# maxsonate/video-diffusion-nnx

Measured on AMD Instinct MI355X. Metric: denoised frames/sec, 16fx64x64 1000-step DDPM, higher is better.
Workload: dtype bf16; 1 GPU; config_v2_2 (north-star shape): Unet3D dim=64 C=1, 16f x 64x64, DDPM T=1000 p_sample_loop (UNet forward + p_sample per step, hipGraph replay); value = n_gpus*B*F/(T*s_per_step); batch_per_gpu=64, parallelism=dp1 (independent samples, no collective), mfma_operands=bf16, storage=weights fp32 master, activations bf16, fp32 accumulate, process_group=none (single process)

## Files before the change

video_diffusion_nnx_amd/csrc/attention.hip:

```cpp
#include "vdx_common.h"
#include <type_traits>
#include "vdx_internal.h"
#include <stdlib.h>
#include <algorithm>

namespace vdx {

template <int MODE, int LP, int TMO>
__global__ __launch_bounds__(256) void attention_kernel(const AttnArgs P) {
    using M = Mma<MODE>;
    constexpr int KT = M::KT, KC = M::KC, RS = ROW_STRIDE;
    constexpr int APIECES = KT / 4;
    constexpr int NSEQ = 64 / LP, QT = LP / 16;
    constexpr int NCHD = 32 / KC;
    constexpr int NCHL = (LP + KC - 1) / KC;
    constexpr int RSV = NCHL * 64 + 16;
    constexpr int D = 32;

    extern __shared__ __attribute__((aligned(16))) char smem[];
    long* rowoff = reinterpret_cast<long*>(smem);
    char* xs = smem + 512;
    char* ws = xs + 64 * RS;
    char* qs = ws + 96 * RS;
    char* ks = qs + 64 * RS;
// ... 462 lines not shown
            for (int b = 0; b < SB; ++b)
#pragma unroll
                for (int t = 0; t < 2; ++t) { aq[b][t] = bq[t]; ak[b][t] = bk[t]; av[b][t] = bv[t]; }
#pragma unroll
            for (int b = 0; b < SB; ++b)
#pragma unroll
                for (int kt = 0; kt < NKT; ++kt)
#pragma unroll
                    for (int ch = 0; ch < (TNO == 1 ? 1 : 2); ++ch) {
                        const uint4 xf = *reinterpret_cast<const uint4*>(xs + kt * PLANE + ((s0 + b) * 16 + lp) * RS + ch * 64 + q * 16);
#pragma unroll
                        for (int t = 0; t < 2; ++t) {
                            M::mma(aq[b][t], wf[kt][ch][0][t], xf);
                            M::mma(ak[b][t], wf[kt][ch][1][t], xf);
                            M::mma(av[b][t], xf, wf[kt][ch][2][t]);
                        }
                    }
            f32x4 sc[SB];
#pragma unroll
            for (int b = 0; b < SB; ++b) {
                sc[b] = f32x4{0.f, 0.f, 0.f, 0.f};
                core_mma16<M, F8>(sc[b], ak[b][0], aq[b][0]);
                core_mma16<M, F8>(sc[b], ak[b][1], aq[b][1]);
            }
            float mx[SB], sum[SB];
#pragma unroll
            for (int b = 0; b < SB; ++b) {
                if (masked) {
#pragma unroll
                    for (int r = 0; r < 4; ++r) if (4 * q + r >= seq_len) sc[b][r] = -1e30f;
                }
                mx[b] = fmaxf(fmaxf(sc[b][0], sc[b][1]), fmaxf(sc[b][2], sc[b][3]));
            }
#pragma unroll
            for (int b = 0; b < SB; ++b) mx[b] = max_q(mx[b]);
#pragma unroll
            for (int b = 0; b < SB; ++b) {
                const float nmx = -mx[b] * escale;
                sum[b] = 0.f;
#pragma unroll
                for (int r = 0; r < 4; ++r) { sc[b][r] = __builtin_amdgcn_exp2f(fmaf(sc[b][r], escale, nmx)); sum[b] += sc[b][r]; }
            }
#pragma unroll
            for (int b = 0; b < SB; ++b) sum[b] = reduce_q(sum[b]);
#pragma unroll
            for (int b = 0; b < SB; ++b) {
                const float inv = __builtin_amdgcn_rcpf(sum[b]);
#pragma unroll
                for (int r = 0; r < 4; ++r) sc[b][r] *= inv;
            }
#pragma unroll
            for (int b = 0; b < SB; ++b) {
                f32x4 o[2];
#pragma unroll
                for (int t = 0; t < 2; ++t) {
                    o[t] = f32x4{0.f, 0.f, 0.f, 0.f};
                    core_mma16<M, F8>(o[t], av[b][t], sc[b]);
                }
                char* orow = os_w + ((s0 + b) * 16 + lp) * RSO;
                if constexpr (OSP) {
                    *reinterpret_cast<uint4*>(orow + h * D * 2 + q * 16) =
                        make_uint4(pack_bf16x2(o[0][0], o[0][1]), pack_bf16x2(o[0][2], o[0][3]), pack_bf16x2(o[1][0], o[1][1]), pack_bf16x2(o[1][2], o[1][3]));
                } else {
#pragma unroll
                    for (int t = 0; t < 2; ++t) M::store4(orow, h * D + t * 16 + 4 * q, make_float4(o[t][0], o[t][1], o[t][2], o[t][3]));
                }
            }
        }
    };
    auto phase_b = [&](const char* os_r, char* ys_w) __attribute__((always_inline)) {
        f32x4 oacc[TMO][TNO];
#pragma unroll
        for (int i = 0; i < TMO; ++i)
#pragma unroll
            for (int j = 0; j < TNO; ++j) oacc[i][j] = bo[i];
#pragma unroll
        for (int ch = 0; ch < NCHO; ++ch) {
// ... 98 lines not shown
    auto kfn = attention_h8_kernel<MODE, NKT, TMO, TNO, IO16, F8, FULL>;
    if (hipError_t e = lds_opt_in(kfn, lds); e != hipSuccess) return e;
    const long subtiles = (a.nseq + 3) / 4;
    const int nsub_cap = 32;
    const int nsub = (int)std::min<long>(nsub_cap, std::max<long>(1, subtiles / 1024));
    const long blocks = (subtiles + nsub - 1) / nsub;
    const AttnWork aw = attn_work(a, M::ES, true);
    LaunchScope ls(st, "attention_h8_kernel", aw.flops, aw.bytes, "<%d, %d, %d, %d, %d, %d, %d> C%d L%d nseq%ld", MODE, NKT, TMO, TNO, (int)IO16, (int)F8, (int)FULL, a.C, a.L, a.nseq);
    hipLaunchKernelGGL(kfn, dim3((unsigned)blocks), dim3(512), lds, st, a, nsub);
    return hipGetLastError();
}

#ifndef VDX_AW_SKEW
#define VDX_AW_SKEW 40
#endif
#ifndef VDX_AW_PRIO
#define VDX_AW_PRIO 1
#endif
#ifndef VDX_AW_SB
#define VDX_AW_SB 4
#endif
#ifndef VDX_AW_NW
#define VDX_AW_NW 8
#endif
template <bool F8, int C = 64, bool FULL = true>
__global__ __launch_bounds__(64 * VDX_AW_NW) void attention_w_kernel(const AttnArgs P, const int groups_per_wave, const long ngroups) {
    using M = Mma<MODE_BF16>;
    constexpr int HD = 256, D = 32, SB = VDX_AW_SB, NT = 64 * VDX_AW_NW;
    constexpr int NCH = C / 32, NTL = C / 16;
    static_assert(C == 64 || C == 32, "C");
    extern __shared__ __attribute__((aligned(16))) char smem[];
    char* Wq = smem;
    char* Wo = Wq + 3 * HD * 128;
    float* bl = reinterpret_cast<float*>(Wo + C * 512);
    const int tid = threadIdx.x, lane = tid & 63;
    const int wave_u = __builtin_amdgcn_readfirstlane(tid >> 6);
    const int lp = lane & 15, q = lane >> 4;

    for (int i = tid; i < 3 * HD * 8; i += NT) {
        const int r = i >> 3, c = i & 7;
        *reinterpret_cast<uint4*>(Wq + r * 128 + 16 * (c ^ (r & 7))) = *reinterpret_cast<const uint4*>(reinterpret_cast<const char*>(P.wqkv) + (size_t)r * 128 + c * 16);
    }
    for (int i = tid; i < C * 32; i += NT) {
        const int R = i >> 5, c = i & 31, hh = c >> 2, qq = c & 3;
        const int tile = R >> 4, ri = R & 15;
        const int co = 32 * (tile >> 1) + 8 * (ri >> 2) + 4 * (tile & 1) + (ri & 3);
        const char* src = reinterpret_cast<const char*>(P.wo) + (size_t)co * 512 + hh * 64 + qq * 8;
        const uint2 lo = *reinterpret_cast<const uint2*>(src), hi = *reinterpret_cast<const uint2*>(src + 32);
        *reinterpret_cast<uint4*>(Wo + R * 512 + 16 * (c ^ (R & 15))) = make_uint4(lo.x, lo.y, hi.x, hi.y);
    }
    for (int i = tid; i < 3 * HD; i += NT) bl[i] = P.bqkv[i];
    if (tid < C) bl[3 * HD + tid] = P.bo[tid];
    __syncthreads();

    const long g_first = ((long)blockIdx.x * VDX_AW_NW + wave_u) * groups_per_wave;
    const long g_end = g_first + groups_per_wave < ngroups ? g_first + groups_per_wave : ngroups;
    if (g_first >= g_end) return;
#if VDX_AW_SKEW
    if (wave_u >= 4) __builtin_amdgcn_s_sleep(VDX_AW_SKEW);
    if (wave_u >= 8) __builtin_amdgcn_s_sleep(VDX_AW_SKEW);
#endif
    const char* const xg = reinterpret_cast<const char*>(P.x);
    char* const yg = reinterpret_cast<char*>(P.y);
    const unsigned loff = (unsigned)(lp * P.tok_stride + q * 8) * 2u;
    const bool tok_ok = FULL || lp < P.L;
    const unsigned sstr = (unsigned)P.inner_stride * 2u;
    auto group_base = [&](long g) __attribute__((always_inline)) -> size_t {
        const unsigned inner = (unsigned)P.inner, sg0 = (unsigned)(g * SB);
        return ((size_t)(sg0 / inner) * P.outer_stride + (size_t)(sg0 % inner) * P.inner_stride) * 2;
    };
    uint4 xn[SB][NCH];
    auto fetch = [&](long g) __attribute__((always_inline)) {
        const char* p = xg + group_base(g) + loff;
#pragma unroll
        for (int b = 0; b < SB; ++b)
#pragma unroll
            for (int ch = 0; ch < NCH; ++ch) {
                xn[b][ch] = make_uint4(0u, 0u, 0u, 0u);
                if (tok_ok) xn[b][ch] = *reinterpret_cast<const uint4*>(p + b * sstr + ch * 64);
            }
    };
    const float escale = P.scale * 1.44269504088896f;
    int wqo[2];
#pragma unroll
    for (int ch = 0; ch < 2; ++ch) wqo[ch] = lp * 128 + 16 * ((ch * 4 + q) ^ (lp & 7));
    const int woo = lp * 512;

    uint4 wcur[2][2], wnext[2][2];
#pragma unroll
    for (int t = 0; t < 2; ++t)
#pragma unroll
        for (int ch = 0; ch < 2; ++ch) wcur[ch][t] = *reinterpret_cast<const uint4*>(Wq + t * 16 * 128 + wqo[ch]);
    fetch(g_first);
    for (long g = g_first; g < g_end; ++g) {
        uint4 xc[SB][NCH];
#pragma unroll
        for (int b = 0; b < SB; ++b)
#pragma unroll
            for (int ch = 0; ch < NCH; ++ch) xc[b][ch] = xn[b][ch];
        if (g + 1 < g_end) fetch(g + 1);
        f32x4 oacc[SB][NTL];
#pragma unroll
        for (int tile = 0; tile < NTL; ++tile) {
            const float4 b4 = *reinterpret_cast<const float4*>(bl + 3 * HD + 32 * (tile >> 1) + 8 * q + 4 * (tile & 1));
#pragma unroll
            for (int b = 0; b < SB; ++b) oacc[b][tile] = f32x4{b4.x, b4.y, b4.z, b4.w};
        }
#pragma unroll 1
        for (int h = 0; h < 8; ++h) {
            const char* wh = Wq + h * (D * 128);
            auto rd = [&](uint4 (&w)[2][2], const char* base) __attribute__((always_inline)) {
#pragma unroll
                for (int t = 0; t < 2; ++t)
#pragma unroll
                    for (int ch = 0; ch < NCH; ++ch) w[ch][t] = *reinterpret_cast<const uint4*>(base + t * 16 * 128 + wqo[ch]);
            };
            f32x4 aq[SB][2], ak[SB][2], av[SB][2];
#pragma unroll
            for (int t = 0; t < 2; ++t) {
                const float4 b4 = *reinterpret_cast<const float4*>(bl + h * D + t * 16 + 4 * q);
#pragma unroll
                for (int b = 0; b < SB; ++b) aq[b][t] = f32x4{b4.x, b4.y, b4.z, b4.w};
            }
            rd(wnext, wh + HD * 128);
            __builtin_amdgcn_sched_barrier(0);
            if (VDX_AW_PRIO) __builtin_amdgcn_s_setprio(1);
#pragma unroll
            for (int ch = 0; ch < NCH; ++ch)
#pragma unroll
                for (int t = 0; t < 2; ++t)
#pragma unroll
                    for (int b = 0; b < SB; ++b) M::mma(aq[b][t], wcur[ch][t], xc[b][ch]);
#pragma unroll
            for (int t = 0; t < 2; ++t) {
                const float4 b4 = *reinterpret_cast<const float4*>(bl + HD + h * D + t * 16 + 4 * q);
#pragma unroll
                for (int b = 0; b < SB; ++b) ak[b][t] = f32x4{b4.x, b4.y, b4.z, b4.w};
            }
            __builtin_amdgcn_sched_barrier(0);
            rd(wcur, wh + 2 * HD * 128);
            __builtin_amdgcn_sched_barrier(0);
#pragma unroll
            for (int ch = 0; ch < NCH; ++ch)
#pragma unroll
                for (int t = 0; t < 2; ++t)
#pragma unroll
                    for (int b = 0; b < SB; ++b) M::mma(ak[b][t], wnext[ch][t], xc[b][ch]);
            f32x4 sc[SB];
#pragma unroll
            for (int b = 0; b < SB; ++b) {
                sc[b] = f32x4{0.f, 0.f, 0.f, 0.f};
                core_mma16<M, F8>(sc[b], ak[b][0], aq[b][0]);
                core_mma16<M, F8>(sc[b], ak[b][1], aq[b][1]);
            }
            if constexpr (!FULL) {
#pragma unroll
                for (int b = 0; b < SB; ++b)
#pragma unroll
                    for (int r = 0; r < 4; ++r) if (4 * q + r >= P.L) sc[b][r] = -1e30f;
            }
#pragma unroll
            for (int t = 0; t < 2; ++t) {
                const float c = bl[2 * HD + h * D + t * 16 + lp];
#pragma unroll
                for (int b = 0; b < SB; ++b) av[b][t] = f32x4{c, c, c, c};
            }
            __builtin_amdgcn_sched_barrier(0);
            {
                const char* woh = Wo + woo + 16 * ((4 * h + q) ^ lp);
#pragma unroll
                for (int tile = 0; tile < NTL; ++tile) wnext[tile >> 1][tile & 1] = *reinterpret_cast<const uint4*>(woh + tile * 8192);
            }
            __builtin_amdgcn_sched_barrier(0);
#pragma unroll
            for (int ch = 0; ch < NCH; ++ch)
#pragma unroll
                for (int t = 0; t < 2; ++t)
#pragma unroll
                    for (int b = 0; b < SB; ++b) M::mma(av[b][t], xc[b][ch], wcur[ch][t]);
            if (VDX_AW_PRIO) __builtin_amdgcn_s_setprio(0);
            float mx[SB], sum[SB];
#pragma unroll
            for (int b = 0; b < SB; ++b) mx[b] = fmaxf(fmaxf(sc[b][0], sc[b][1]), fmaxf(sc[b][2], sc[b][3]));
#pragma unroll
            for (int b = 0; b < SB; ++b) mx[b] = max_q(mx[b]);
#pragma unroll
            for (int b = 0; b < SB; ++b) {
                const float nmx = -mx[b] * escale;
                sum[b] = 0.f;
#pragma unroll
                for (int r = 0; r < 4; ++r) { sc[b][r] = __builtin_amdgcn_exp2f(fmaf(sc[b][r], escale, nmx)); sum[b] += sc[b][r]; }
            }
#pragma unroll
            for (int b = 0; b < SB; ++b) sum[b] = reduce_q(sum[b]);
#pragma unroll
            for (int b = 0; b < SB; ++b) {
                const float inv = __builtin_amdgcn_rcpf(sum[b]);
#pragma unroll
                for (int r = 0; r < 4; ++r) sc[b][r] *= inv;
            }
            __builtin_amdgcn_sched_barrier(0);
            rd(wcur, Wq + ((h + 1) & 7) * (D * 128));
            f32x4 o[SB][2];
#pragma unroll
            for (int b = 0; b < SB; ++b)
#pragma unroll
                for (int t = 0; t < 2; ++t) {
                    o[b][t] = f32x4{0.f, 0.f, 0.f, 0.f};
                    core_mma16<M, F8>(o[b][t], av[b][t], sc[b]);
                }
            __builtin_amdgcn_sched_barrier(0);
            uint4 of[SB];
#pragma unroll
            for (int b = 0; b < SB; ++b)
                of[b] = make_uint4(pack_bf16x2(o[b][0][0], o[b][0][1]), pack_bf16x2(o[b][0][2], o[b][0][3]), pack_bf16x2(o[b][1][0], o[b][1][1]), pack_bf16x2(o[b][1][2], o[b][1][3]));
#pragma unroll
            for (int tile = 0; tile < NTL; ++tile)
#pragma unroll
                for (int b = 0; b < SB; ++b) M::mma(oacc[b][tile], wnext[tile >> 1][tile & 1], of[b]);
        }
        char* yp = yg + group_base(g) + loff;
#pragma unroll
        for (int b = 0; b < SB; ++b)
#pragma unroll
            for (int wc = 0; wc < NCH; ++wc) {
                const uint4 r = xc[b][wc];
                const f32x4 a0 = oacc[b][2 * wc], a1 = oacc[b][2 * wc + 1];
                uint4 w;
                w.x = pack_bf16x2(a0[0] + __uint_as_float(r.x << 16), a0[1] + __uint_as_float(r.x & 0xFFFF0000u));
                w.y = pack_bf16x2(a0[2] + __uint_as_float(r.y << 16), a0[3] + __uint_as_float(r.y & 0xFFFF0000u));
                w.z = pack_bf16x2(a1[0] + __uint_as_float(r.z << 16), a1[1] + __uint_as_float(r.z & 0xFFFF0000u));
                w.w = pack_bf16x2(a1[2] + __uint_as_float(r.w << 16), a1[3] + __uint_as_float(r.w & 0xFFFF0000u));
                if (tok_ok) *reinterpret_cast<uint4*>(yp + b * sstr + wc * 64) = w;
            }
    }
}

static bool attn_w_eligible(const AttnArgs& a) {
    return a.io_bf16 && (a.C == 64 || a.C == 32) && a.CPad == 64 && a.HDPad == 256 && a.heads == 8 && a.L >= 1 && a.L <= 16 && a.inner % 4 == 0 &&
           a.nseq % 4 == 0 && a.nseq >= 256 && a.nseq < (1L << 29) && 3 * a.inner_stride + 15 * a.tok_stride + a.C < (1L << 30);
}
template <bool F8>
static hipError_t launch_attn_w(const AttnArgs& a, hipStream_t st) {
    const size_t lds = 3 * 256 * 128 + (size_t)a.C * 512 + (3 * 256 + 64) * 4;
    const long ngroups = a.nseq / VDX_AW_SB;
    const PersistentSplit s = persistent_split(ngroups, (long)device_cus() * VDX_AW_NW);
    const int gpw = (int)s.per;
    const long blocks = (s.workers + VDX_AW_NW - 1) / VDX_AW_NW;
    const AttnWork aw = attn_work(a, 2, true);
    auto go = [&](auto kfn) -> hipError_t {
        if (hipError_t e = lds_opt_in(kfn, lds); e != hipSuccess) return e;
        LaunchScope ls(st, "attention_w_kernel", aw.flops, aw.bytes, "<fp8 %d> C%d L%d nseq%ld", (int)F8, a.C, a.L, a.nseq);
        hipLaunchKernelGGL(kfn, dim3((unsigned)blocks), dim3(64 * VDX_AW_NW), lds, st, a, gpw, ngroups);
        return hipGetLastError();
    };
    if (a.C == 64) return a.L == 16 ? go(attention_w_kernel<F8, 64, true>) : go(attention_w_kernel<F8, 64, false>);
    return a.L == 16 ? go(attention_w_kernel<F8, 32, true>) : go(attention_w_kernel<F8, 32, false>);
}

template <bool IO16, int TT, bool F8, int LT = 1>
__global__ __launch_bounds__(512) void attention_head_kernel(const AttnArgs P, const int seq_per_block, const int nchunks) {
    using M = Mma<MODE_BF16>;
    constexpr int D = 32, NS = TT / LT;
    static_assert(TT % LT == 0, "whole sequences per group");
    extern __shared__ __attribute__((aligned(16))) char smem[];
    const int tid = threadIdx.x, lane = tid & 63, w = tid >> 6;
    const int lp = lane & 15, q = lane >> 4;
    const int h = (blockIdx.x >> 3) & 7, HD = P.heads * D;
    const int chunk_id = (blockIdx.x >> 6) * 8 + (blockIdx.x & 7);
    if (chunk_id >= nchunks) return;
    const int RSW = P.C * 2 + 32;
    const int cpr = P.C / 8;
    for (int i = tid; i < 96 * cpr; i += 512) {
        const int row = i / cpr, pc = i - row * cpr;
        const int part = row >> 5, rr = row & 31;
        *reinterpret_cast<uint4*>(smem + row * RSW + pc * 16) = *reinterpret_cast<const uint4*>(
            reinterpret_cast<const char*>(P.wqkv) + ((size_t)(part * HD + h * D + rr) * P.CPad) * 2 + pc * 16);
// ... 286 lines not shown
```

video_diffusion_nnx_amd/csrc/sla.hip:

```cpp
#include "vdx_common.h"
#include "vdx_internal.h"
#include <stdlib.h>

namespace vdx {

constexpr int SLA_PART = 32 * 32 + 64;

template <int MODE>
__global__ __launch_bounds__(256) void sla_ctx_kernel(const SlaArgs P) {
    using M = Mma<MODE>;
    constexpr int KT = M::KT, KC = M::KC, RS = ROW_STRIDE;
    constexpr int APIECES = KT / 4;
    constexpr int NCHN = 64 / KC;
    constexpr int RSE = NCHN * 64 + 16;

    extern __shared__ __attribute__((aligned(16))) char smem[];
    float* m_run = reinterpret_cast<float*>(smem);
    float* s_run = m_run + 32;
    float* alpha = s_run + 32;
    float* pm = alpha + 32;
    char* xs = smem + 1024;
    char* ws = xs + 64 * RS;
    char* eT = ws + 64 * RS;
    char* vT = eT + 32 * RSE;
// ... 321 lines not shown
    using M = Mma<MODE>;
    static_assert(!IO16 || MODE == MODE_BF16, "bf16 activation storage implies bf16 MFMA operands");
    static constexpr int PCH = IO16 ? 8 : 4;
    static constexpr int APIECES = M::KT / PCH;
    static constexpr int XP = 64 * APIECES * NKT / 512;
    static constexpr int PLANE = 64 * ROW_STRIDE;
    static constexpr int BUF = NKT * PLANE;
    float4 xpre[XP];
    __device__ __forceinline__ void fetch(const float* x, size_t xbase, int io_bf16, int r0, int N, int C, int tid) {
#pragma unroll
        for (int u = 0; u < XP; ++u) {
            const int i = tid + 512 * u;
            const int kt = i / (64 * APIECES), rem = i % (64 * APIECES);
            const int row = rem / APIECES, c = kt * M::KT + (rem % APIECES) * PCH;
            xpre[u] = make_float4(0.f, 0.f, 0.f, 0.f);
            if (r0 + row < N && c < C) {
                if (IO16) xpre[u] = *reinterpret_cast<const float4*>(reinterpret_cast<const char*>(x) + (xbase + (size_t)(r0 + row) * C + c) * 2);
                else xpre[u] = load4_f32_or_bf16(x, xbase + (size_t)(r0 + row) * C + c, io_bf16);
            }
        }
    }
    __device__ __forceinline__ void put(char* xs, int tid) const {
#pragma unroll
        for (int u = 0; u < XP; ++u) {
            const int i = tid + 512 * u;
            const int kt = i / (64 * APIECES), rem = i % (64 * APIECES);
            char* dst = xs + kt * PLANE + (rem / APIECES) * ROW_STRIDE;
            if (IO16) *reinterpret_cast<float4*>(dst + (rem % APIECES) * 16) = xpre[u];
            else M::store4(dst, (rem % APIECES) * 4, xpre[u]);
        }
    }
};

template <bool FULL>
__device__ __forceinline__ void ctx8_softmax_step(f32x4 (&acc)[2][4], float (&m_run)[2], float (&s_run)[2], f32x4 (&cacc)[2][2], int nleft) {
    constexpr float L2E = 1.44269504088896f;
#pragma unroll
    for (int dt = 0; dt < 2; ++dt) {
        if (!FULL) {
#pragma unroll
            for (int tn = 0; tn < 2; ++tn)
#pragma unroll
                for (int r = 0; r < 4; ++r) if (tn * 16 + r >= nleft) acc[tn][dt][r] = -1e30f;
        }
        float mx = fmaxf(fmaxf(fmaxf(acc[0][dt][0], acc[0][dt][1]), fmaxf(acc[0][dt][2], acc[0][dt][3])),
                         fmaxf(fmaxf(acc[1][dt][0], acc[1][dt][1]), fmaxf(acc[1][dt][2], acc[1][dt][3])));
        mx = max_q(mx);
        const float mn = fmaxf(m_run[dt], mx);
        const float alpha = __builtin_amdgcn_exp2f((m_run[dt] - mn) * L2E);
        m_run[dt] = mn;
        const float nb = -mn * L2E;
        float ssum = 0.f;
#pragma unroll
        for (int tn = 0; tn < 2; ++tn)
#pragma unroll
            for (int r = 0; r < 4; ++r) {
                float e = __builtin_amdgcn_exp2f(__builtin_fmaf(acc[tn][dt][r], L2E, nb));
                if (!FULL) e = (tn * 16 + r >= nleft) ? 0.f : e;
                acc[tn][dt][r] = e;
                ssum += e;
            }
        s_run[dt] = s_run[dt] * alpha + reduce_q(ssum);
#pragma unroll
        for (int et = 0; et < 2; ++et)
#pragma unroll
            for (int r = 0; r < 4; ++r) cacc[et][dt][r] *= alpha;
    }
}

template <int MODE, int NKT, bool IO16>
__global__ __launch_bounds__(512) void sla_ctx8_kernel(const SlaArgs P) {
    using M = Mma<MODE>;
    using T = SlaTile<MODE, NKT, IO16>;
    constexpr int RS = ROW_STRIDE;
    extern __shared__ __attribute__((aligned(16))) char smem[];
    const int tid = threadIdx.x, lane = tid & 63, h = tid >> 6;
    const int lp = lane & 15, q = lane >> 4;
    const int n = blockIdx.x / P.nchunk, chunk = blockIdx.x % P.nchunk;
    const int R = P.nsub * 64;
    const size_t xbase = (size_t)n * P.N * P.C;

    uint4 wf[NKT][2][4];
#pragma unroll
    for (int kt = 0; kt < NKT; ++kt)
#pragma unroll
        for (int ch = 0; ch < 2; ++ch)
#pragma unroll
            for (int tm = 0; tm < 4; ++tm) {
                const char* base = reinterpret_cast<const char*>(tm < 2 ? P.wk : P.wv);
                wf[kt][ch][tm] = *reinterpret_cast<const uint4*>(base + ((size_t)(h * 32 + (tm & 1) * 16 + lp) * P.CPad + kt * M::KT) * M::ES + ch * 64 + q * 16);
            }
    float m_run[2] = {-1e30f, -1e30f}, s_run[2] = {0.f, 0.f};
    f32x4 cacc[2][2];
#pragma unroll
    for (int i = 0; i < 2; ++i) { cacc[i][0] = f32x4{0.f, 0.f, 0.f, 0.f}; cacc[i][1] = f32x4{0.f, 0.f, 0.f, 0.f}; }

    T t;
    t.fetch(P.x, xbase, P.io_bf16, chunk * R, P.N, P.C, tid);
    t.put(smem, tid);
    __syncthreads();
    for (int sub = 0; sub < P.nsub; ++sub) {
        const int r0 = chunk * R + sub * 64;
        if (r0 >= P.N) break;
        const char* xs = smem + (sub & 1) * T::BUF;
        const bool more = (sub + 1 < P.nsub) && (r0 + 64 < P.N);
        if (more) t.fetch(P.x, xbase, P.io_bf16, r0 + 64, P.N, P.C, tid);
#pragma unroll
        for (int hf = 0; hf < 2; ++hf) {
            f32x4 acc[2][4];
#pragma unroll
            for (int i = 0; i < 2; ++i)
#pragma unroll
                for (int j = 0; j < 4; ++j) acc[i][j] = f32x4{0.f, 0.f, 0.f, 0.f};
#pragma unroll
            for (int kt = 0; kt < NKT; ++kt)
#pragma unroll
                for (int ch = 0; ch < 2; ++ch) {
                    uint4 xa[2];
#pragma unroll
                    for (int tn = 0; tn < 2; ++tn)
                        xa[tn] = *reinterpret_cast<const uint4*>(xs + kt * T::PLANE + ((hf * 2 + tn) * 16 + lp) * RS + ch * 64 + q * 16);
#pragma unroll
                    for (int tn = 0; tn < 2; ++tn)
#pragma unroll
                        for (int tm = 0; tm < 4; ++tm) M::mma(acc[tn][tm], xa[tn], wf[kt][ch][tm]);
                }
            if (r0 + 64 <= P.N) ctx8_softmax_step<true>(acc, m_run, s_run, cacc, 0);
            else ctx8_softmax_step<false>(acc, m_run, s_run, cacc, P.N - (r0 + hf * 32 + 4 * q));
#pragma unroll
            for (int tn = 0; tn < 2; ++tn)
#pragma unroll
                for (int et = 0; et < 2; ++et)
#pragma unroll
                    for (int dt = 0; dt < 2; ++dt) M::mma16(cacc[et][dt], acc[tn][2 + et], acc[tn][dt]);
        }
        if (more) t.put(smem + ((sub + 1) & 1) * T::BUF, tid);
        __syncthreads();
    }
    if (P.nchunk == 1) {
        char* ct = reinterpret_cast<char*>(P.ctxT) + (size_t)(n * P.heads + h) * 32 * 32 * M::ES;
#pragma unroll
        for (int dt = 0; dt < 2; ++dt) {
            const float inv = 1.0f / s_run[dt];
#pragma unroll
            for (int et = 0; et < 2; ++et)
#pragma unroll
                for (int r = 0; r < 4; ++r) M::store1(ct + (size_t)(et * 16 + 4 * q + r) * 32 * M::ES, dt * 16 + lp, cacc[et][dt][r] * inv);
        }
        return;
    }
    float* part = P.part + ((size_t)(n * P.nchunk + chunk) * P.heads + h) * SLA_PART;
#pragma unroll
    for (int et = 0; et < 2; ++et)
#pragma unroll
        for (int dt = 0; dt < 2; ++dt)
            *reinterpret_cast<float4*>(part + (dt * 16 + lp) * 32 + et * 16 + 4 * q) =
                make_float4(cacc[et][dt][0], cacc[et][dt][1], cacc[et][dt][2], cacc[et][dt][3]);
    if (q == 0) {
#pragma unroll
        for (int dt = 0; dt < 2; ++dt) { part[1024 + dt * 16 + lp] = m_run[dt]; part[1056 + dt * 16 + lp] = s_run[dt]; }
    }
}

template <int MODE, int NKT, int TMO, int TNO, bool IO16>
__global__ __launch_bounds__(512, NKT == 1 ? 4 : 2) void sla_out8_kernel(const SlaArgs P) {
    using M = Mma<MODE>;
    using T = SlaTile<MODE, NKT, IO16>;
// ... 180 lines not shown

    for (int i = tid; i < HD * 8; i += 512) {
        const int r = i >> 3, c = i & 7;
        *reinterpret_cast<uint4*>(Wq + r * 128 + 16 * (c ^ (r & 7))) = *reinterpret_cast<const uint4*>(reinterpret_cast<const char*>(P.wq) + (size_t)r * 128 + c * 16);
    }
    for (int i = tid; i < 64 * 32; i += 512) {
        const int R = i >> 5, c = i & 31, hh = c >> 2, qq = c & 3;
        const int tile = R >> 4, ri = R & 15;
        const int co = 32 * (tile >> 1) + 8 * (ri >> 2) + 4 * (tile & 1) + (ri & 3);
        const char* src = reinterpret_cast<const char*>(P.wo) + (size_t)co * 512 + hh * 64 + qq * 8;
        const uint2 lo = *reinterpret_cast<const uint2*>(src), hi = *reinterpret_cast<const uint2*>(src + 32);
        *reinterpret_cast<uint4*>(Wo + R * 512 + 16 * (c ^ (R & 15))) = make_uint4(lo.x, lo.y, hi.x, hi.y);
    }
    auto load_ctx = [&](int f, int par) __attribute__((always_inline)) {
        const char* src = reinterpret_cast<const char*>(P.ctxT) + (size_t)f * (8 * 32 * 32 * 2);
        uint4 v[2];
#pragma unroll
        for (int u = 0; u < 2; ++u) v[u] = *reinterpret_cast<const uint4*>(src + (size_t)(tid + 512 * u) * 16);
#pragma unroll
        for (int u = 0; u < 2; ++u) {
            const int i = tid + 512 * u, row = i >> 2, pc = i & 3;
            char* d = Cx + par * (256 * CRS) + row * CRS + pc * 16;
            *reinterpret_cast<uint2*>(d) = make_uint2(v[u].x, v[u].y);
            *reinterpret_cast<uint2*>(d + 8) = make_uint2(v[u].z, v[u].w);
        }
    };
    load_ctx(f0, 0);
    __syncthreads();

    const int gpf = P.N >> 6;
    const char* const xg = reinterpret_cast<const char*>(P.x);
    char* const yg = reinterpret_cast<char*>(P.y);
    const unsigned loff = (unsigned)(lp * 64 + q * 8) * 2u;
    int wqo[2];
#pragma unroll
    for (int ch = 0; ch < 2; ++ch) wqo[ch] = lp * 128 + 16 * ((ch * 4 + q) ^ (lp & 7));
    const int woo = lp * 512;

    uint4 xn[4][2];
    auto fetch = [&](int f, int g) __attribute__((always_inline)) {
        const char* p = xg + ((size_t)f * P.N + (size_t)g * 64) * 128 + loff;
#pragma unroll
        for (int tn = 0; tn < 4; ++tn)
#pragma unroll
            for (int ch = 0; ch < 2; ++ch) xn[tn][ch] = *reinterpret_cast<const uint4*>(p + tn * (16 * 128) + ch * 64);
    };
    uint4 wcur[2][2], wnext[2][2];
    auto rd = [&](uint4 (&w)[2][2], const char* base) __attribute__((always_inline)) {
#pragma unroll
        for (int t = 0; t < 2; ++t)
#pragma unroll
            for (int ch = 0; ch < 2; ++ch) w[ch][t] = *reinterpret_cast<const uint4*>(base + t * 16 * 128 + wqo[ch]);
    };
    rd(wcur, Wq);
    if (wave_u < gpf) fetch(f0, wave_u);
    for (int f = f0; f < f1; ++f) {
        const int par = (f - f0) & 1;
        if (f + 1 < f1) load_ctx(f + 1, par ^ 1);
        const char* cimg = Cx + par * (256 * CRS);
        for (int g = wave_u; g < gpf; g += 8) {
            uint4 xc[4][2];
#pragma unroll
            for (int tn = 0; tn < 4; ++tn) { xc[tn][0] = xn[tn][0]; xc[tn][1] = xn[tn][1]; }
            if (g + 8 < gpf) fetch(f, g + 8);
            else if (f + 1 < f1 && wave_u < gpf) fetch(f + 1, wave_u);
            f32x4 yacc[4][4];
#pragma unroll
            for (int tn = 0; tn < 4; ++tn)
#pragma unroll
                for (int tile = 0; tile < 4; ++tile) yacc[tn][tile] = f32x4{0.f, 0.f, 0.f, 0.f};
#pragma unroll 1
            for (int h = 0; h < 8; ++h) {
                f32x4 acc[2][4];
#pragma unroll
                for (int i = 0; i < 2; ++i)
#pragma unroll
                    for (int j = 0; j < 4; ++j) acc[i][j] = f32x4{0.f, 0.f, 0.f, 0.f};
                {
                    const char* woh = Wo + woo + 16 * ((4 * h + q) ^ lp);
#pragma unroll
                    for (int tile = 0; tile < 4; ++tile) wnext[tile >> 1][tile & 1] = *reinterpret_cast<const uint4*>(woh + tile * 8192);
                }
                __builtin_amdgcn_sched_barrier(0);
#pragma unroll
                for (int ch = 0; ch < 2; ++ch)
#pragma unroll
                    for (int tm = 0; tm < 2; ++tm)
#pragma unroll
                        for (int tn = 0; tn < 4; ++tn) M::mma(acc[tm][tn], wcur[ch][tm], xc[tn][ch]);
                uint2 cf[2][2];
#pragma unroll
                for (int et = 0; et < 2; ++et)
#pragma unroll
                    for (int dt = 0; dt < 2; ++dt) cf[et][dt] = *reinterpret_cast<const uint2*>(cimg + (h * 32 + et * 16 + lp) * CRS + dt * 32 + q * 8);
                __builtin_amdgcn_sched_barrier(0);
                rd(wcur, Wq + ((h + 1) & 7) * (32 * 128));
#pragma unroll
                for (int tn = 0; tn < 4; ++tn) {
                    float mx = -1e30f;
#pragma unroll
                    for (int tm = 0; tm < 2; ++tm)
#pragma unroll
                        for (int r = 0; r < 4; ++r) mx = fmaxf(mx, acc[tm][tn][r]);
                    mx = max_q(mx);
                    const float nmx = -mx * 1.44269504088896f;
                    float sum = 0.f;
#pragma unroll
                    for (int tm = 0; tm < 2; ++tm)
#pragma unroll
                        for (int r = 0; r < 4; ++r) { acc[tm][tn][r] = __builtin_amdgcn_exp2f(fmaf(acc[tm][tn][r], 1.44269504088896f, nmx)); sum += acc[tm][tn][r]; }
                    const float inv = __builtin_amdgcn_rcpf(reduce_q(sum));
#pragma unroll
                    for (int tm = 0; tm < 2; ++tm)
#pragma unroll
                        for (int r = 0; r < 4; ++r) acc[tm][tn][r] *= inv;
                }
                uint4 of[4];
#pragma unroll
                for (int tn = 0; tn < 4; ++tn) {
                    f32x4 o[2];
#pragma unroll
                    for (int et = 0; et < 2; ++et) {
                        o[et] = f32x4{0.f, 0.f, 0.f, 0.f};
#pragma unroll
                        for (int dt = 0; dt < 2; ++dt) {
                            const uint2 qb = make_uint2(pack_bf16x2(acc[dt][tn][0], acc[dt][tn][1]), pack_bf16x2(acc[dt][tn][2], acc[dt][tn][3]));
                            o[et] = __builtin_amdgcn_mfma_f32_16x16x16bf16_1k(__builtin_bit_cast(s16x4, cf[et][dt]), __builtin_bit_cast(s16x4, qb), o[et], 0, 0, 0);
                        }
                    }
                    of[tn] = make_uint4(pack_bf16x2(o[0][0], o[0][1]), pack_bf16x2(o[0][2], o[0][3]), pack_bf16x2(o[1][0], o[1][1]), pack_bf16x2(o[1][2], o[1][3]));
                }
#pragma unroll
                for (int tile = 0; tile < 4; ++tile)
#pragma unroll
                    for (int tn = 0; tn < 4; ++tn) M::mma(yacc[tn][tile], wnext[tile >> 1][tile & 1], of[tn]);
            }
            char* yp = yg + ((size_t)f * P.N + (size_t)g * 64) * 128 + loff;
#pragma unroll
            for (int tn = 0; tn < 4; ++tn)
#pragma unroll
                for (int wc = 0; wc < 2; ++wc) {
                    const uint4 r = xc[tn][wc];
                    const f32x4 a0 = yacc[tn][2 * wc], a1 = yacc[tn][2 * wc + 1];
                    uint4 w;
// ... 334 lines not shown
```

video_diffusion_nnx_amd/csrc/vdx_common.h:

```cpp
#pragma once
#include <hip/hip_runtime.h>
#include <stdint.h>

namespace vdx {

enum { MODE_F32 = 0, MODE_BF16 = 1, MODE_F16 = 2 };

typedef float f32x4 __attribute__((ext_vector_type(4)));
typedef float f32x2 __attribute__((ext_vector_type(2)));
typedef __bf16 bf16x8 __attribute__((ext_vector_type(8)));
typedef __bf16 bf16x2 __attribute__((ext_vector_type(2)));
typedef short s16x4 __attribute__((ext_vector_type(4)));

constexpr int CHUNK_BYTES = 64;
constexpr int ROW_BYTES = 128;
constexpr int ROW_STRIDE = 160;
constexpr float NORM_EPS = 1e-6f;
constexpr int GN_SLOTS = 32;

__device__ __forceinline__ unsigned pack_bf16x2(float a, float b) {
    f32x2 v = {a, b};
    bf16x2 r = __builtin_convertvector(v, bf16x2);
    return __builtin_bit_cast(unsigned, r);
}
// ... 111 lines not shown
    if (!is_bf16) return *reinterpret_cast<const float4*>(base + i);
    const uint2 u = *reinterpret_cast<const uint2*>(reinterpret_cast<const char*>(base) + i * 2);
    return make_float4(__uint_as_float(u.x << 16), __uint_as_float(u.x & 0xFFFF0000u), __uint_as_float(u.y << 16), __uint_as_float(u.y & 0xFFFF0000u));
}

__device__ __forceinline__ void store4_f32_or_bf16(float* base, size_t i, float4 v, int is_bf16) {
    if (!is_bf16) *reinterpret_cast<float4*>(base + i) = v;
    else *reinterpret_cast<uint2*>(reinterpret_cast<char*>(base) + i * 2) = make_uint2(pack_bf16x2(v.x, v.y), pack_bf16x2(v.z, v.w));
}

template <int CTRL>
__device__ __forceinline__ float dpp_row(float v) {
    return __uint_as_float(__builtin_amdgcn_update_dpp(0u, __float_as_uint(v), CTRL, 0xF, 0xF, true));
}
__device__ __forceinline__ float reduce16(float v) {
    v += dpp_row<0xB1>(v);
    v += dpp_row<0x4E>(v);
    v += dpp_row<0x141>(v);
    v += dpp_row<0x140>(v);
    return v;
}
__device__ __forceinline__ float reduce_q(float v) {
    const auto a = __builtin_amdgcn_permlane32_swap(__float_as_uint(v), __float_as_uint(v), false, false);
    v = __uint_as_float(a[0]) + __uint_as_float(a[1]);
    const auto b = __builtin_amdgcn_permlane16_swap(__float_as_uint(v), __float_as_uint(v), false, false);
    return __uint_as_float(b[0]) + __uint_as_float(b[1]);
}
__device__ __forceinline__ float max_q(float v) {
    const auto a = __builtin_amdgcn_permlane32_swap(__float_as_uint(v), __float_as_uint(v), false, false);
    v = fmaxf(__uint_as_float(a[0]), __uint_as_float(a[1]));
    const auto b = __builtin_amdgcn_permlane16_swap(__float_as_uint(v), __float_as_uint(v), false, false);
    return fmaxf(__uint_as_float(b[0]), __uint_as_float(b[1]));
}
__device__ __forceinline__ float max16(float v) {
    v = fmaxf(v, dpp_row<0xB1>(v));
    v = fmaxf(v, dpp_row<0x4E>(v));
    v = fmaxf(v, dpp_row<0x141>(v));
    v = fmaxf(v, dpp_row<0x140>(v));
    return v;
}
__device__ __forceinline__ int div_magic(int n, unsigned m) { return (int)__umulhi((unsigned)n, m); }

__device__ __forceinline__ void gn_mean_rstd(const double* stats, int b, int g, int groups, double count,
                                             float& mean, float& rstd) {
    double s = 0.0, ss = 0.0;
    const double* p = stats + (size_t)b * GN_SLOTS * groups * 2 + g * 2;
    static_assert(GN_SLOTS % 8 == 0, "GN_SLOTS");
#pragma unroll 1
    for (int k0 = 0; k0 < GN_SLOTS; k0 += 8) {
        double2 t[8];
#pragma unroll
        for (int k = 0; k < 8; ++k) t[k] = *reinterpret_cast<const double2*>(p + (size_t)(k0 + k) * groups * 2);
#pragma unroll
        for (int k = 0; k < 8; ++k) { s += t[k].x; ss += t[k].y; }
    }
    double m = s / count;
    double var = ss / count - m * m;
    if (var < 0.0) var = 0.0;
    mean = (float)m;
    rstd = (float)(1.0 / sqrt(var + (double)NORM_EPS));
}

__device__ __forceinline__ void gn_mean_rstd_wg(const double* stats, int b, int groups, double count, float* gm, int tid, int nthreads) {
    static_assert(GN_SLOTS == 32, "GN_SLOTS");
    for (int t = tid; t < groups * GN_SLOTS; t += nthreads) {
        const int g = t >> 5, slot = t & 31;
        const double2 v = *reinterpret_cast<const double2*>(stats + (((size_t)b * GN_SLOTS + slot) * groups + g) * 2);
        double s = v.x, ss = v.y;
#pragma unroll
        for (int o = 16; o >= 1; o >>= 1) { s += __shfl_xor(s, o); ss += __shfl_xor(ss, o); }
        if (slot == 0) {
            const double m = s / count;
// ... 16 lines not shown
```

Baseline: 48.06 frames/s.

## Batch cross-lane softmax reductions, use incremental LDS pointers, skip unchanged online-softmax rescale

```diff
diff --git a/video_diffusion_nnx_amd/csrc/attention.hip b/video_diffusion_nnx_amd/csrc/attention.hip
--- a/video_diffusion_nnx_amd/csrc/attention.hip
+++ b/video_diffusion_nnx_amd/csrc/attention.hip
@@ -518,8 +518,7 @@
                 }
                 mx[b] = fmaxf(fmaxf(sc[b][0], sc[b][1]), fmaxf(sc[b][2], sc[b][3]));
             }
-#pragma unroll
-            for (int b = 0; b < SB; ++b) mx[b] = max_q(mx[b]);
+            max_qn(mx);
 #pragma unroll
             for (int b = 0; b < SB; ++b) {
                 const float nmx = -mx[b] * escale;
@@ -527,8 +526,7 @@
 #pragma unroll
                 for (int r = 0; r < 4; ++r) { sc[b][r] = __builtin_amdgcn_exp2f(fmaf(sc[b][r], escale, nmx)); sum[b] += sc[b][r]; }
             }
-#pragma unroll
-            for (int b = 0; b < SB; ++b) sum[b] = reduce_q(sum[b]);
+            reduce_qn(sum);
 #pragma unroll
             for (int b = 0; b < SB; ++b) {
                 const float inv = __builtin_amdgcn_rcpf(sum[b]);
@@ -693,14 +691,16 @@
     extern __shared__ __attribute__((aligned(16))) char smem[];
     char* Wq = smem;
     char* Wo = Wq + 3 * HD * 128;
-    float* bl = reinterpret_cast<float*>(Wo + C * 512);
+    char* bl = Wo + C * 512;
+    constexpr int BHS = 2 * D * 4 + D * 16, BO0 = 8 * BHS;
     const int tid = threadIdx.x, lane = tid & 63;
     const int wave_u = __builtin_amdgcn_readfirstlane(tid >> 6);
     const int lp = lane & 15, q = lane >> 4;
 
     for (int i = tid; i < 3 * HD * 8; i += NT) {
         const int r = i >> 3, c = i & 7;
-        *reinterpret_cast<uint4*>(Wq + r * 128 + 16 * (c ^ (r & 7))) = *reinterpret_cast<const uint4*>(reinterpret_cast<const char*>(P.wqkv) + (size_t)r * 128 + c * 16);
+        const int rl = ((r >> 5) & 7) * 96 + (r >> 8) * 32 + (r & 31);
+        *reinterpret_cast<uint4*>(Wq + rl * 128 + 16 * (c ^ (r & 7))) = *reinterpret_cast<const uint4*>(reinterpret_cast<const char*>(P.wqkv) + (size_t)r * 128 + c * 16);
     }
     for (int i = tid; i < C * 32; i += NT) {
         const int R = i >> 5, c = i & 31, hh = c >> 2, qq = c & 3;
@@ -710,8 +710,13 @@
         const uint2 lo = *reinterpret_cast<const uint2*>(src), hi = *reinterpret_cast<const uint2*>(src + 32);
         *reinterpret_cast<uint4*>(Wo + R * 512 + 16 * (c ^ (R & 15))) = make_uint4(lo.x, lo.y, hi.x, hi.y);
     }
-    for (int i = tid; i < 3 * HD; i += NT) bl[i] = P.bqkv[i];
-    if (tid < C) bl[3 * HD + tid] = P.bo[tid];
+    for (int i = tid; i < 3 * HD; i += NT) {
+        const int part = i >> 8, hh = (i >> 5) & 7, d = i & 31;
+        const float c = P.bqkv[i];
+        if (part < 2) *reinterpret_cast<float*>(bl + hh * BHS + part * (D * 4) + d * 4) = c;
+        else *reinterpret_cast<float4*>(bl + hh * BHS + 2 * D * 4 + d * 16) = make_float4(c, c, c, c);
+    }
+    if (tid < C) *reinterpret_cast<float*>(bl + BO0 + tid * 4) = P.bo[tid];
     __syncthreads();
 
     const long g_first = ((long)blockIdx.x * VDX_AW_NW + wave_u) * groups_per_wave;
@@ -742,16 +747,20 @@
             }
     };
     const float escale = P.scale * 1.44269504088896f;
-    int wqo[2];
-#pragma unroll
-    for (int ch = 0; ch < 2; ++ch) wqo[ch] = lp * 128 + 16 * ((ch * 4 + q) ^ (lp & 7));
-    const int woo = lp * 512;
+    constexpr int HSTR = 3 * D * 128, WO0 = 3 * HD * 128, BL0 = WO0 + C * 512;
+    const unsigned lds0 = lds_addr(smem);
+    unsigned pw[2], pwo = lds0 + WO0 + lp * 512 + 16 * (q ^ lp), pbq = lds0 + BL0 + 16 * q, pbv = lds0 + BL0 + 2 * D * 4 + 16 * lp;
+#pragma unroll
+    for (int ch = 0; ch < 2; ++ch) pw[ch] = lds0 + lp * 128 + 16 * ((ch * 4 + q) ^ (lp & 7));
+    auto rd = [&](uint4 (&w)[2][2], int off) __attribute__((always_inline)) {
+#pragma unroll
+        for (int t = 0; t < 2; ++t)
+#pragma unroll
+            for (int ch = 0; ch < NCH; ++ch) w[ch][t] = lds_ld<uint4>(pw[ch] + (off + t * 16 * 128));
+    };
 
     uint4 wcur[2][2], wnext[2][2];
-#pragma unroll
-    for (int t = 0; t < 2; ++t)
-#pragma unroll
-        for (int ch = 0; ch < 2; ++ch) wcur[ch][t] = *reinterpret_cast<const uint4*>(Wq + t * 16 * 128 + wqo[ch]);
+    rd(wcur, 0);
     fetch(g_first);
     for (long g = g_first; g < g_end; ++g) {
         uint4 xc[SB][NCH];
@@ -763,27 +772,20 @@
         f32x4 oacc[SB][NTL];
 #pragma unroll
         for (int tile = 0; tile < NTL; ++tile) {
-            const float4 b4 = *reinterpret_cast<const float4*>(bl + 3 * HD + 32 * (tile >> 1) + 8 * q + 4 * (tile & 1));
+            const float4 b4 = *reinterpret_cast<const float4*>(bl + BO0 + (32 * (tile >> 1) + 8 * q + 4 * (tile & 1)) * 4);
 #pragma unroll
             for (int b = 0; b < SB; ++b) oacc[b][tile] = f32x4{b4.x, b4.y, b4.z, b4.w};
         }
 #pragma unroll 1
         for (int h = 0; h < 8; ++h) {
-            const char* wh = Wq + h * (D * 128);
-            auto rd = [&](uint4 (&w)[2][2], const char* base) __attribute__((always_inline)) {
-#pragma unroll
-                for (int t = 0; t < 2; ++t)
-#pragma unroll
-                    for (int ch = 0; ch < NCH; ++ch) w[ch][t] = *reinterpret_cast<const uint4*>(base + t * 16 * 128 + wqo[ch]);
-            };
             f32x4 aq[SB][2], ak[SB][2], av[SB][2];
 #pragma unroll
             for (int t = 0; t < 2; ++t) {
-                const float4 b4 = *reinterpret_cast<const float4*>(bl + h * D + t * 16 + 4 * q);
+                const float4 b4 = lds_ld<float4>(pbq + t * 64);
 #pragma unroll
                 for (int b = 0; b < SB; ++b) aq[b][t] = f32x4{b4.x, b4.y, b4.z, b4.w};
             }
-            rd(wnext, wh + HD * 128);
+            rd(wnext, D * 128);
             __builtin_amdgcn_sched_barrier(0);
             if (VDX_AW_PRIO) __builtin_amdgcn_s_setprio(1);
 #pragma unroll
@@ -794,12 +796,12 @@
                     for (int b = 0; b < SB; ++b) M::mma(aq[b][t], wcur[ch][t], xc[b][ch]);
 #pragma unroll
             for (int t = 0; t < 2; ++t) {
-                const float4 b4 = *reinterpret_cast<const float4*>(bl + HD + h * D + t * 16 + 4 * q);
+                const float4 b4 = lds_ld<float4>(pbq + (D * 4 + t * 64));
 #pragma unroll
                 for (int b = 0; b < SB; ++b) ak[b][t] = f32x4{b4.x, b4.y, b4.z, b4.w};
             }
             __builtin_amdgcn_sched_barrier(0);
-            rd(wcur, wh + 2 * HD * 128);
+            rd(wcur, 2 * D * 128);
             __builtin_amdgcn_sched_barrier(0);
 #pragma unroll
             for (int ch = 0; ch < NCH; ++ch)
@@ -822,15 +824,14 @@
             }
 #pragma unroll
             for (int t = 0; t < 2; ++t) {
-                const float c = bl[2 * HD + h * D + t * 16 + lp];
-#pragma unroll
-                for (int b = 0; b < SB; ++b) av[b][t] = f32x4{c, c, c, c};
+                const float4 c4 = lds_ld<float4>(pbv + t * 256);
+#pragma unroll
+                for (int b = 0; b < SB; ++b) av[b][t] = f32x4{c4.x, c4.y, c4.z, c4.w};
             }
             __builtin_amdgcn_sched_barrier(0);
             {
-                const char* woh = Wo + woo + 16 * ((4 * h + q) ^ lp);
-#pragma unroll
-                for (int tile = 0; tile < NTL; ++tile) wnext[tile >> 1][tile & 1] = *reinterpret_cast<const uint4*>(woh + tile * 8192);
+#pragma unroll
+                for (int tile = 0; tile < NTL; ++tile) wnext[tile >> 1][tile & 1] = lds_ld<uint4>(pwo + tile * 8192);
             }
             __builtin_amdgcn_sched_barrier(0);
 #pragma unroll
@@ -843,8 +844,7 @@
             float mx[SB], sum[SB];
 #pragma unroll
             for (int b = 0; b < SB; ++b) mx[b] = fmaxf(fmaxf(sc[b][0], sc[b][1]), fmaxf(sc[b][2], sc[b][3]));
-#pragma unroll
-            for (int b = 0; b < SB; ++b) mx[b] = max_q(mx[b]);
+            max_qn(mx);
 #pragma unroll
             for (int b = 0; b < SB; ++b) {
                 const float nmx = -mx[b] * escale;
@@ -852,8 +852,7 @@
 #pragma unroll
                 for (int r = 0; r < 4; ++r) { sc[b][r] = __builtin_amdgcn_exp2f(fmaf(sc[b][r], escale, nmx)); sum[b] += sc[b][r]; }
             }
-#pragma unroll
-            for (int b = 0; b < SB; ++b) sum[b] = reduce_q(sum[b]);
+            reduce_qn(sum);
 #pragma unroll
             for (int b = 0; b < SB; ++b) {
                 const float inv = __builtin_amdgcn_rcpf(sum[b]);
@@ -861,7 +860,16 @@
                 for (int r = 0; r < 4; ++r) sc[b][r] *= inv;
             }
             __builtin_amdgcn_sched_barrier(0);
-            rd(wcur, Wq + ((h + 1) & 7) * (D * 128));
+            {
+                const bool last = h == 7;
+                const int dw = last ? -7 * HSTR : HSTR, db = last ? -7 * BHS : BHS;
+#pragma unroll
+                for (int ch = 0; ch < NCH; ++ch) pw[ch] += dw;
+                pwo ^= (unsigned)((h ^ (h + 1)) & 7) << 6;
+                pbq += db; pbv += db;
+                asm volatile("" : "+v"(pw[0]), "+v"(pw[1]), "+v"(pwo), "+v"(pbq), "+v"(pbv));
+            }
+            rd(wcur, 0);
             f32x4 o[SB][2];
 #pragma unroll
             for (int b = 0; b < SB; ++b)
@@ -903,7 +911,7 @@
 }
 template <bool F8>
 static hipError_t launch_attn_w(const AttnArgs& a, hipStream_t st) {
-    const size_t lds = 3 * 256 * 128 + (size_t)a.C * 512 + (3 * 256 + 64) * 4;
+    const size_t lds = 3 * 256 * 128 + (size_t)a.C * 512 + 8 * (2 * 32 * 4 + 32 * 16) + 64 * 4;
     const long ngroups = a.nseq / VDX_AW_SB;
     const PersistentSplit s = persistent_split(ngroups, (long)device_cus() * VDX_AW_NW);
     const int gpw = (int)s.per;
diff --git a/video_diffusion_nnx_amd/csrc/sla.hip b/video_diffusion_nnx_amd/csrc/sla.hip
--- a/video_diffusion_nnx_amd/csrc/sla.hip
+++ b/video_diffusion_nnx_amd/csrc/sla.hip
@@ -377,9 +377,12 @@
     }
 };
 
+#ifndef VDX_CTX8_SKIP
+#define VDX_CTX8_SKIP 1
+#endif
 template <bool FULL>
-__device__ __forceinline__ void ctx8_softmax_step(f32x4 (&acc)[2][4], float (&m_run)[2], float (&s_run)[2], f32x4 (&cacc)[2][2], int nleft) {
-    constexpr float L2E = 1.44269504088896f;
+__device__ __forceinline__ void ctx8_step_max(f32x4 (&acc)[2][4], float (&mx)[2], int nleft) {
+    if (!FULL) asm volatile("" : "+v"(nleft));
 #pragma unroll
     for (int dt = 0; dt < 2; ++dt) {
         if (!FULL) {
@@ -388,29 +391,26 @@
 #pragma unroll
                 for (int r = 0; r < 4; ++r) if (tn * 16 + r >= nleft) acc[tn][dt][r] = -1e30f;
         }
-        float mx = fmaxf(fmaxf(fmaxf(acc[0][dt][0], acc[0][dt][1]), fmaxf(acc[0][dt][2], acc[0][dt][3])),
-                         fmaxf(fmaxf(acc[1][dt][0], acc[1][dt][1]), fmaxf(acc[1][dt][2], acc[1][dt][3])));
-        mx = max_q(mx);
-        const float mn = fmaxf(m_run[dt], mx);
-        const float alpha = __builtin_amdgcn_exp2f((m_run[dt] - mn) * L2E);
-        m_run[dt] = mn;
-        const float nb = -mn * L2E;
-        float ssum = 0.f;
-#pragma unroll
-        for (int tn = 0; tn < 2; ++tn)
-#pragma unroll
-            for (int r = 0; r < 4; ++r) {
-                float e = __builtin_amdgcn_exp2f(__builtin_fmaf(acc[tn][dt][r], L2E, nb));
-                if (!FULL) e = (tn * 16 + r >= nleft) ? 0.f : e;
-                acc[tn][dt][r] = e;
-                ssum += e;
-            }
-        s_run[dt] = s_run[dt] * alpha + reduce_q(ssum);
-#pragma unroll
-        for (int et = 0; et < 2; ++et)
-#pragma unroll
-            for (int r = 0; r < 4; ++r) cacc[et][dt][r] *= alpha;
-    }
+        mx[dt] = fmaxf(fmaxf(fmaxf(acc[0][dt][0], acc[0][dt][1]), fmaxf(acc[0][dt][2], acc[0][dt][3])),
+                       fmaxf(fmaxf(acc[1][dt][0], acc[1][dt][1]), fmaxf(acc[1][dt][2], acc[1][dt][3])));
+    }
+    max_qn(mx);
+}
+template <bool FULL>
+__device__ __forceinline__ float ctx8_step_exp(f32x4 (&acc)[2][4], int dt, float mn, int nleft) {
+    if (!FULL) asm volatile("" : "+v"(nleft));
+    const float nb = -mn * 1.44269504088896f;
+    float ssum = 0.f;
+#pragma unroll
+    for (int tn = 0; tn < 2; ++tn)
+#pragma unroll
+        for (int r = 0; r < 4; ++r) {
+            float e = __builtin_amdgcn_exp2f(__builtin_fmaf(acc[tn][dt][r], 1.44269504088896f, nb));
+            if (!FULL) e = (tn * 16 + r >= nleft) ? 0.f : e;
+            acc[tn][dt][r] = e;
+            ssum += e;
+        }
+    return reduce_q(ssum);
 }
 
 template <int MODE, int NKT, bool IO16>
@@ -470,14 +470,32 @@
 #pragma unroll
                         for (int tm = 0; tm < 4; ++tm) M::mma(acc[tn][tm], xa[tn], wf[kt][ch][tm]);
                 }
-            if (r0 + 64 <= P.N) ctx8_softmax_step<true>(acc, m_run, s_run, cacc, 0);
-            else ctx8_softmax_step<false>(acc, m_run, s_run, cacc, P.N - (r0 + hf * 32 + 4 * q));
-#pragma unroll
-            for (int tn = 0; tn < 2; ++tn)
-#pragma unroll
-                for (int et = 0; et < 2; ++et)
-#pragma unroll
-                    for (int dt = 0; dt < 2; ++dt) M::mma16(cacc[et][dt], acc[tn][2 + et], acc[tn][dt]);
+            const bool full = r0 + 64 <= P.N;
+            const int nleft = P.N - (r0 + hf * 32 + 4 * q);
+            float mx[2];
+            if (full) ctx8_step_max<true>(acc, mx, 0); else ctx8_step_max<false>(acc, mx, nleft);
+#pragma unroll
+            for (int dt = 0; dt < 2; ++dt) {
+                const float mn = fmaxf(m_run[dt], mx[dt]);
+                const bool moved = !VDX_CTX8_SKIP || __builtin_amdgcn_ballot_w64(mn != m_run[dt]) != 0;
+                const float dm = (m_run[dt] - mn) * 1.44269504088896f;
+                m_run[dt] = mn;
+                const float ssum = full ? ctx8_step_exp<true>(acc, dt, mn, 0) : ctx8_step_exp<false>(acc, dt, mn, nleft);
+                auto mm = [&](f32x4& c0, f32x4& c1) __attribute__((always_inline)) {
+#pragma unroll
+                    for (int tn = 0; tn < 2; ++tn) { M::mma16(c0, acc[tn][2], acc[tn][dt]); M::mma16(c1, acc[tn][3], acc[tn][dt]); }
+                };
+                if (moved) {
+                    const float alpha = __builtin_amdgcn_exp2f(dm);
+                    s_run[dt] = s_run[dt] * alpha + ssum;
+                    f32x4 c0 = cacc[0][dt] * alpha, c1 = cacc[1][dt] * alpha;
+                    mm(c0, c1);
+                    cacc[0][dt] = c0; cacc[1][dt] = c1;
+                } else {
+                    s_run[dt] = s_run[dt] + ssum;
+                    mm(cacc[0][dt], cacc[1][dt]);
+                }
+            }
         }
         if (more) t.put(smem + ((sub + 1) & 1) * T::BUF, tid);
         __syncthreads();
@@ -724,10 +742,10 @@
     const char* const xg = reinterpret_cast<const char*>(P.x);
     char* const yg = reinterpret_cast<char*>(P.y);
     const unsigned loff = (unsigned)(lp * 64 + q * 8) * 2u;
-    int wqo[2];
-#pragma unroll
-    for (int ch = 0; ch < 2; ++ch) wqo[ch] = lp * 128 + 16 * ((ch * 4 + q) ^ (lp & 7));
-    const int woo = lp * 512;
+    const unsigned lds0 = lds_addr(smem);
+    unsigned pw[2], pwo = lds0 + HD * 128 + lp * 512 + 16 * (q ^ lp), pcx = 0;
+#pragma unroll
+    for (int ch = 0; ch < 2; ++ch) pw[ch] = lds0 + lp * 128 + 16 * ((ch * 4 + q) ^ (lp & 7));
 
     uint4 xn[4][2];
     auto fetch = [&](int f, int g) __attribute__((always_inline)) {
@@ -738,18 +756,18 @@
             for (int ch = 0; ch < 2; ++ch) xn[tn][ch] = *reinterpret_cast<const uint4*>(p + tn * (16 * 128) + ch * 64);
     };
     uint4 wcur[2][2], wnext[2][2];
-    auto rd = [&](uint4 (&w)[2][2], const char* base) __attribute__((always_inline)) {
+    auto rd = [&](uint4 (&w)[2][2]) __attribute__((always_inline)) {
 #pragma unroll
         for (int t = 0; t < 2; ++t)
 #pragma unroll
-            for (int ch = 0; ch < 2; ++ch) w[ch][t] = *reinterpret_cast<const uint4*>(base + t * 16 * 128 + wqo[ch]);
+            for (int ch = 0; ch < 2; ++ch) w[ch][t] = lds_ld<uint4>(pw[ch] + t * 16 * 128);
     };
-    rd(wcur, Wq);
+    rd(wcur);
     if (wave_u < gpf) fetch(f0, wave_u);
     for (int f = f0; f < f1; ++f) {
         const int par = (f - f0) & 1;
         if (f + 1 < f1) load_ctx(f + 1, par ^ 1);
-        const char* cimg = Cx + par * (256 * CRS);
+        pcx = lds0 + 2 * HD * 128 + par * (256 * CRS) + lp * CRS + q * 8;
         for (int g = wave_u; g < gpf; g += 8) {
             uint4 xc[4][2];
 #pragma unroll
@@ -768,11 +786,8 @@
                 for (int i = 0; i < 2; ++i)
 #pragma unroll
                     for (int j = 0; j < 4; ++j) acc[i][j] = f32x4{0.f, 0.f, 0.f, 0.f};
-                {
-                    const char* woh = Wo + woo + 16 * ((4 * h + q) ^ lp);
-#pragma unroll
-                    for (int tile = 0; tile < 4; ++tile) wnext[tile >> 1][tile & 1] = *reinterpret_cast<const uint4*>(woh + tile * 8192);
-                }
+#pragma unroll
+                for (int tile = 0; tile < 4; ++tile) wnext[tile >> 1][tile & 1] = lds_ld<uint4>(pwo + tile * 8192);
                 __builtin_amdgcn_sched_barrier(0);
 #pragma unroll
                 for (int ch = 0; ch < 2; ++ch)
@@ -784,24 +799,40 @@
 #pragma unroll
                 for (int et = 0; et < 2; ++et)
 #pragma unroll
-                    for (int dt = 0; dt < 2; ++dt) cf[et][dt] = *reinterpret_cast<const uint2*>(cimg + (h * 32 + et * 16 + lp) * CRS + dt * 32 + q * 8);
+                    for (int dt = 0; dt < 2; ++dt) cf[et][dt] = lds_ld<uint2>(pcx + (et * 16 * CRS + dt * 32));
                 __builtin_amdgcn_sched_barrier(0);
-                rd(wcur, Wq + ((h + 1) & 7) * (32 * 128));
+                {
+                    const bool last = h == 7;
+                    const int dw = last ? -7 * 32 * 128 : 32 * 128, dc = last ? -7 * 32 * CRS : 32 * CRS;
+                    pw[0] += dw; pw[1] += dw;
+                    pwo ^= (unsigned)((h ^ (h + 1)) & 7) << 6;
+                    pcx += dc;
+                    asm volatile("" : "+v"(pw[0]), "+v"(pw[1]), "+v"(pwo), "+v"(pcx));
+                }
+                rd(wcur);
+                float mx[4], sum[4];
 #pragma unroll
                 for (int tn = 0; tn < 4; ++tn) {
-                    float mx = -1e30f;
+                    mx[tn] = -1e30f;
 #pragma unroll
                     for (int tm = 0; tm < 2; ++tm)
 #pragma unroll
-                        for (int r = 0; r < 4; ++r) mx = fmaxf(mx, acc[tm][tn][r]);
-                    mx = max_q(mx);
-                    const float nmx = -mx * 1.44269504088896f;
-                    float sum = 0.f;
+                        for (int r = 0; r < 4; ++r) mx[tn] = fmaxf(mx[tn], acc[tm][tn][r]);
+                }
+                max_qn(mx);
+#pragma unroll
+                for (int tn = 0; tn < 4; ++tn) {
+                    const float nmx = -mx[tn] * 1.44269504088896f;
+                    sum[tn] = 0.f;
 #pragma unroll
                     for (int tm = 0; tm < 2; ++tm)
 #pragma unroll
-                        for (int r = 0; r < 4; ++r) { acc[tm][tn][r] = __builtin_amdgcn_exp2f(fmaf(acc[tm][tn][r], 1.44269504088896f, nmx)); sum += acc[tm][tn][r]; }
-                    const float inv = __builtin_amdgcn_rcpf(reduce_q(sum));
+                        for (int r = 0; r < 4; ++r) { acc[tm][tn][r] = __builtin_amdgcn_exp2f(fmaf(acc[tm][tn][r], 1.44269504088896f, nmx)); sum[tn] += acc[tm][tn][r]; }
+                }
+                reduce_qn(sum);
+#pragma unroll
+                for (int tn = 0; tn < 4; ++tn) {
+                    const float inv = __builtin_amdgcn_rcpf(sum[tn]);
 #pragma unroll
                     for (int tm = 0; tm < 2; ++tm)
 #pragma unroll
diff --git a/video_diffusion_nnx_amd/csrc/vdx_common.h b/video_diffusion_nnx_amd/csrc/vdx_common.h
--- a/video_diffusion_nnx_amd/csrc/vdx_common.h
+++ b/video_diffusion_nnx_amd/csrc/vdx_common.h
@@ -167,12 +167,71 @@
     const auto b = __builtin_amdgcn_permlane16_swap(__float_as_uint(v), __float_as_uint(v), false, false);
     return fmaxf(__uint_as_float(b[0]), __uint_as_float(b[1]));
 }
+#ifndef VDX_QSWAP_MULTI
+#define VDX_QSWAP_MULTI 1
+#endif
+struct QAdd { static __device__ __forceinline__ float op(float a, float b) { return a + b; } static __device__ __forceinline__ float one(float v) { return reduce_q(v); } };
+struct QMax { static __device__ __forceinline__ float op(float a, float b) { return fmaxf(a, b); } static __device__ __forceinline__ float one(float v) { return max_q(v); } };
+template <class OP> __device__ __forceinline__ float q_fold32(float x, float y) {
+    const auto a = __builtin_amdgcn_permlane32_swap(__float_as_uint(x), __float_as_uint(y), false, false);
+    return OP::op(__uint_as_float(a[0]), __uint_as_float(a[1]));
+}
+template <class OP> __device__ __forceinline__ float q_fold16(float x, float y) {
+    const auto a = __builtin_amdgcn_permlane16_swap(__float_as_uint(x), __float_as_uint(y), false, false);
+    return OP::op(__uint_as_float(a[0]), __uint_as_float(a[1]));
+}
+__device__ __forceinline__ void q_spread16(float x, float& even, float& odd) {
+    const auto a = __builtin_amdgcn_permlane16_swap(__float_as_uint(x), __float_as_uint(x), false, false);
+    even = __uint_as_float(a[0]); odd = __uint_as_float(a[1]);
+}
+__device__ __forceinline__ void q_spread32(float x, float& lo, float& hi) {
+    const auto a = __builtin_amdgcn_permlane32_swap(__float_as_uint(x), __float_as_uint(x), false, false);
+    lo = __uint_as_float(a[0]); hi = __uint_as_float(a[1]);
+}
+template <class OP> __device__ __forceinline__ void q4(float (&v)[4]) {
+#if VDX_QSWAP_MULTI
+    const float s = q_fold16<OP>(q_fold32<OP>(v[0], v[1]), q_fold32<OP>(v[2], v[3]));
+    float e, o;
+    q_spread16(s, e, o);
+    q_spread32(e, v[0], v[1]);
+    q_spread32(o, v[2], v[3]);
+#else
+#pragma unroll
+    for (int i = 0; i < 4; ++i) v[i] = OP::one(v[i]);
+#endif
+}
+template <class OP> __device__ __forceinline__ void q2(float (&v)[2]) {
+#if VDX_QSWAP_MULTI
+    const float p = q_fold32<OP>(v[0], v[1]);
+    float e, o;
+    q_spread16(p, e, o);
+    q_spread32(OP::op(e, o), v[0], v[1]);
+#else
+    v[0] = OP::one(v[0]); v[1] = OP::one(v[1]);
+#endif
+}
+template <class OP, int N> __device__ __forceinline__ void qn(float (&v)[N]) {
+    if constexpr (N == 4) q4<OP>(v);
+    else if constexpr (N == 2) q2<OP>(v);
+    else {
+#pragma unroll
+        for (int i = 0; i < N; ++i) v[i] = OP::one(v[i]);
+    }
+}
+template <int N> __device__ __forceinline__ void reduce_qn(float (&v)[N]) { qn<QAdd, N>(v); }
+template <int N> __device__ __forceinline__ void max_qn(float (&v)[N]) { qn<QMax, N>(v); }
 __device__ __forceinline__ float max16(float v) {
     v = fmaxf(v, dpp_row<0xB1>(v));
     v = fmaxf(v, dpp_row<0x4E>(v));
     v = fmaxf(v, dpp_row<0x141>(v));
     v = fmaxf(v, dpp_row<0x140>(v));
     return v;
+}
+typedef __attribute__((address_space(3))) char lds_char;
+__device__ __forceinline__ unsigned lds_addr(const void* p) { return (unsigned)(uintptr_t)(const lds_char*)p; }
+template <class T> __device__ __forceinline__ T lds_ld(unsigned a) {
+    typedef unsigned words __attribute__((ext_vector_type(sizeof(T) / 4)));
+    return __builtin_bit_cast(T, *(const __attribute__((address_space(3))) words*)(uintptr_t)a);
 }
 __device__ __forceinline__ int div_magic(int n, unsigned m) { return (int)__umulhi((unsigned)n, m); }
 
```

New measurement: 48.45 frames/s, median of 6. About the same (+0.8%).
